# ch4r10t33r/zigz

Measured on AMD Instinct MI355X. Metric: trace steps/sec proved (BabyBear, 2^20 RV64I trace), higher is better.
Workload: dtype u32

## Files before the change

### zigz_amd/csrc/api_commit.cpp

```cpp
#include "api_internal.hpp"

using namespace zk;
using cp::ListCaps;
static_assert(cp::MAX_LEVELS == RUN_MAX_LEVELS && cp::SUMMARY_WORDS == JOB_SUMMARY_WORDS, "commit_plan.hpp restates kernels.hpp");

static void caps_for(zigz_ctx *ctx, size_t npad, unsigned rn, unsigned gn) {
    ListCaps &c = ctx->caps;
    if (c.npad == npad && c.rn == rn && c.gn == gn) return;
    c.npad = npad;
    c.rn = rn;
    c.gn = gn;
    c.g_slabs = false;
    c.g_drops = c.g_skip = c.g_kept = 0;
    memset(c.r_last, 0, sizeof(c.r_last));
    memset(c.g_last, 0, sizeof(c.g_last));
    c.last_dropped = false;
    const LevelLists rw = runs_lists(npad, rn ? rn : 1), gw = cons_lists(npad);
    for (unsigned l = 0; l < RUN_MAX_LEVELS; l++) {
        c.r[l] = l <= rw.top ? (rw.cap[l] / 8 > 256 ? rw.cap[l] / 8 : 256) : 0;
        c.g[l] = l <= gw.top ? 256 : 0;
    }
}

static TreeRef empty_tree_ref(size_t npad) {
// ... 683 lines not shown
    ZIGZ_NOTHROW_BEGIN
    if (job) ZIGZ_ENTER(job->ctx);
    if (!job || !values || !indices || !leaves) return ZIGZ_ERR_INVALID_ARGUMENT;
    zigz_ctx *ctx = job->ctx;
    if (job->state != 1) return ZIGZ_ERR_BAD_STATE;
    const size_t nv = job->nv, ncols = job->ncols;
    if (nv && (!points || !siblings || !dirs)) return ZIGZ_ERR_INVALID_ARGUMENT;
    const size_t sib_b = ncols * nv * 32, leaf_b = ncols * 4, val_b = ncols * 4, dir_b = ncols * nv;
    const size_t out_b = sib_b + leaf_b + val_b + dir_b;
    if (out_b <= PIN_WORDS * 8 / 2 && nv * ncols * 4 + ncols * 8 <= PIN_WORDS * 8 / 2) {
        uint8_t *h = (uint8_t *)ctx->h_pin;
        uint8_t *z_sib = h;
        uint32_t *z_leaf = (uint32_t *)(h + sib_b), *z_val = z_leaf + ncols;
        uint8_t *z_dirs = (uint8_t *)(z_val + ncols);
        uint64_t *h_idx = ctx->h_pin + PIN_WORDS - ncols;
        for (size_t c = 0; c < ncols; c++) {
            h_idx[c] = nv == 0 ? 0 : points[c * nv] % ((uint64_t)1 << nv);
            indices[c] = h_idx[c];
        }
        const bool arena = job->zstride != 0;
        const bool use = job->facts.run_cols && !job->no_eval_skip && (arena || (job->tree.lists && job->col_stride >= job->N));
        EvalSkip skip;
        if (arena) {
            skip.ncols1 = (unsigned)job->ncols1;
            skip.z_in = job->zstride / 4;
            skip.z_changed = job->zstride / 8;
        }
        if (arena || use) memcpy(skip.y_of_col, job->tree.y_of_col, sizeof(skip.y_of_col));
        const unsigned long long *r_ctr = arena ? (const unsigned long long *)((const uint8_t *)ctx->ws[WS_BATCH] + job->off_r_ctr) : ctx->d_run_count;
        if (use) skip.changed = r_ctr + RUN_CHANGED;
        const size_t n_const = use ? job->const_cols : 0;
        if (arena || use) ctx->stats.eval_constant_columns = n_const;
        CHK(timed_begin(ctx, 4));
        if (arena) CHK(dev_eval_radix(ctx, job->d_cols, job->col_stride, ncols, nv, points, z_val, &skip, n_const));
        else CHK(dev_eval_folds(ctx, job->d_cols, job->col_stride, ncols, nv, points, z_val, use ? &skip : nullptr, n_const));
        CHK(timed_end(ctx, 4, &ctx->stats.eval_us));
        const DoneFlag done = done_flag(ctx, 1);
        launch_paths(job->tree, job->tree.npad, (unsigned)nv, job->d_cols, job->col_stride, h_idx, z_sib, z_dirs, z_leaf,
                     job->zstride ? job->ncols1 : ncols, ctx->stream, done);
        HIPCHK(ctx, hipGetLastError());
        if (!(g_sleep_wait.load() && !ctx->timing && sleep_wait(done.flag, done.seq)))
            HIPCHK(ctx, hipStreamSynchronize(ctx->stream));
        if (sib_b) memcpy(siblings, z_sib, sib_b);
        for (size_t c = 0; c < ncols; c++) {
            leaves[c] = z_leaf[c];
            values[c] = z_val[c];
        }
        if (dir_b) memcpy(dirs, z_dirs, dir_b);
        CHK(bind_pool_collect(ctx));
        job->state = 2;
        return ZIGZ_OK;
    }
    if (job->zstride) {
        set_err(ctx, "batched commit job: the openings do not fit the staging buffer");
        return ZIGZ_ERR_INVALID_ARGUMENT;
    }
    void *dv;
    CHK(ws_get(ctx, WS_SCRATCH, ncols * 4 + 64, &dv));
    CHK(timed_begin(ctx, 4));
    CHK(dev_eval_folds(ctx, job->d_cols, job->col_stride, ncols, nv, points, (uint32_t *)dv));
    CHK(timed_end(ctx, 4, &ctx->stats.eval_us));
    std::vector<uint32_t> hv(ncols);
    HIPCHK(ctx, hipMemcpyAsync(hv.data(), dv, ncols * 4, hipMemcpyDeviceToHost, ctx->stream));
    std::vector<uint64_t> idx(ncols);
    for (size_t c = 0; c < ncols; c++) {
        idx[c] = nv == 0 ? 0 : points[c * nv] % ((uint64_t)1 << nv);
        indices[c] = idx[c];
    }
    CHK(open_paths(ctx, job->tree, (unsigned)nv, job->d_cols, job->col_stride, idx.data(), ncols, siblings, dirs, leaves));
    for (size_t c = 0; c < ncols; c++) values[c] = hv[c];
    CHK(bind_pool_collect(ctx));
    job->state = 2;
// ... 90 lines not shown
```

### zigz_amd/csrc/api_internal.hpp

```cpp
#pragma once
#include "zigz_hip.h"

#include <hip/hip_runtime.h>
#include <stdarg.h>
#include <stdio.h>
#include <stdlib.h>
#include <string.h>
#include <time.h>

#include <atomic>
#include <new>
#include <thread>
#include <vector>

#include "commit_plan.hpp"
#include "field.hpp"
#include "kernels.hpp"
#include "sumcheck_host.hpp"

using namespace zk;

enum { WS_IN64 = 0, WS_IN32, WS_OUT32, WS_OUT64, WS_SCRATCH, WS_TREE, WS_FOLD, WS_MISC, WS_COLS, WS_LASSO, WS_DEDUP, WS_WITNESS, WS_RUNS, WS_RUNMETA, WS_CONS, WS_CONSMETA, WS_BATCH, WS_SCBATCH, WS_SCBATCH_IN, WS_VERIFY, WS_OPEN, WS_MLEBATCH, WS_MLEBATCH_PART, WS_MLEBATCH_IN, WS_PRODUCT, WS_PRODUCT_WORK, WS_PRODUCT_IN, WS_EQ, WS_EQ_OUT, WS_SLOTS };

constexpr int KEV_MAX = 72;
// ... 91 lines not shown
            int d_ = -1;                                                             \
            if (hipGetDevice(&d_) != hipSuccess || d_ != (ctx)->device) (void)hipSetDevice((ctx)->device); \
        }                                                                            \
    } while (0)

inline bool is_pow2(size_t n) { return n && !(n & (n - 1)); }
inline size_t ceil_pow2(size_t n) { size_t v = 1; while (v < n) v <<= 1; return v; }
constexpr size_t align256(size_t b) { return (b + 255) & ~(size_t)255; }


#pragma GCC visibility push(hidden)
void set_err(zigz_ctx *ctx, const char *fmt, ...);
zigz_status ws_get(zigz_ctx *ctx, int slot, size_t bytes, void **out);
bool sleep_wait(const unsigned long long *flag, unsigned long long seq);
bool spin_wait(const unsigned long long *flag, unsigned long long seq);
DoneFlag done_flag(zigz_ctx *ctx, int which);
zigz_status wait_published(zigz_ctx *ctx, const DoneFlag &done);
zigz_status pinned(zigz_ctx *ctx, size_t bytes, uint8_t **out);
zigz_status upload_region(zigz_ctx *ctx, size_t bytes, uint8_t **out);
zigz_status log_launch(zigz_ctx *ctx, int cls, uint64_t perms, hipEvent_t start, hipEvent_t stop, hipEvent_t first, double *dur_us);
zigz_status upload_u64(zigz_ctx *ctx, const uint64_t *h_in, size_t n, uint32_t *d_out, bool reduce);
zigz_status download_u64(zigz_ctx *ctx, const uint32_t *d_in, size_t n, uint64_t *h_out);
uint32_t host_to_mont(uint64_t canonical);
zigz_status read_u64(zigz_ctx *ctx, const void *d_src, size_t words, uint64_t *dst);
zigz_status dev_half_sums(zigz_ctx *ctx, const uint32_t *d_in, size_t n, uint64_t out[2]);
zigz_status timed_begin(zigz_ctx *ctx, int ev);
zigz_status timed_end(zigz_ctx *ctx, int ev, double *us_out);
zigz_status bind_launch(zigz_ctx *ctx, const uint32_t *d_in, size_t in_stride, uint32_t *d_out, size_t out_stride,
                               size_t half, size_t ncols, uint32_t r_m, const uint32_t *d_r_m, unsigned long long *d_sums,
                               const SumsLayout *lay = nullptr);
void bind_pool_reset(zigz_ctx *ctx);
zigz_status bind_pool_collect(zigz_ctx *ctx);
zigz_status dev_eval_radix(zigz_ctx *ctx, const uint32_t *d_cols, size_t col_stride, size_t ncols, size_t nv,
                                  const uint64_t *points, uint32_t *d_vals, const EvalSkip *skip = nullptr, size_t n_const = 0);
zigz_status dev_eval_folds(zigz_ctx *ctx, const uint32_t *d_cols, size_t col_stride, size_t ncols, size_t nv,
                                  const uint64_t *points , uint32_t *d_vals, const EvalSkip *skip = nullptr, size_t n_const = 0);
zigz_status sumcheck_core(zigz_ctx *ctx, const uint32_t *d_in, size_t n, uint32_t *d_scratch,
                                 const uint64_t *fixed, uint64_t *rounds, uint64_t *point, uint64_t *final_eval);
zigz_status stage_in(zigz_ctx *ctx, const uint64_t *in, size_t n, uint32_t **d_out);
zigz_status lasso_mapping_check(const uint64_t *table, size_t table_rows, const uint64_t *queries, size_t n_queries, size_t w,
                                const uint64_t *mapping, size_t n_mapping);
struct BuildHints {
    uint64_t small_domain_mask, run_aware_mask, cons_group_mask;
    bool materialize, job;
};
struct BuildResult {
    TreeRef tree;
    uint64_t run_cols, run_dense, sd_cols, cons_hinted, cons_levels_nodes, cons_sd;
};
zigz_status build_trees(zigz_ctx *ctx, const uint32_t *d_vals, size_t val_stride, size_t n_values, size_t npad,
                               uint8_t *d_slab, size_t ncols, bool record, const BuildHints &in, BuildResult *out);
zigz_status keccak_times_collect(zigz_ctx *ctx);
size_t mle_batch_fill(const uint32_t *const *d_tables, const size_t *ns, size_t k, const uint64_t *points, bool reversed,
                      MleBatchTab *tab, uint32_t *f);
zigz_status stage_host_tables(zigz_ctx *ctx, const uint64_t *const *tables, const size_t *ns, size_t count,
                              const std::vector<size_t> &at, uint32_t *h, int slot, const size_t *owner,
                              std::vector<const uint32_t *> &d, size_t *bad_index);
zigz_status mle_eval_pairs_queue(zigz_ctx *ctx, const void *const *tables, bool host_tables, const size_t *ns, size_t m,
                                 const uint64_t *points, bool reversed, const size_t *owner, const uint64_t **results, DoneFlag *done,
                                 size_t *bad_index);
extern std::atomic<int> g_sleep_wait;
#pragma GCC visibility pop

constexpr const char *NOT_CANONICAL_TEXT = "input contains a value >= p (not a canonical BabyBear element)";
template <class Check>
zigz_status host_checks(zigz_ctx *ctx, const uint64_t *const *tables, const size_t *ns, size_t k, size_t *bad_index, Check check) {
    bool value;
    const zigz_status st = checks_in_call_order(tables, ns, k, bad_index, check, &value);
    if (value) set_err(ctx, "%s", NOT_CANONICAL_TEXT);
// ... 20 lines not shown
```

### zigz_amd/csrc/api_mle.cpp

```cpp
#include "api_internal.hpp"

using namespace zk;

zigz_status dev_half_sums(zigz_ctx *ctx, const uint32_t *d_in, size_t n, uint64_t out[2]) {
    const SumsLayout lay = (aligned16(d_in)) ? half_sums_layout(n, 1, 2048) : SumsLayout{2, 1, 0, 1};
    const size_t words = lay.nslots > 1 || lay.col_stride != 2 ? (size_t)lay.nslots * 32 : 2;
    HIPCHK(ctx, hipMemsetAsync(ctx->d_sums, 0, words * 8, ctx->stream));
    launch_half_sums(d_in, n, n, 1, ctx->d_sums, ctx->stream, nullptr, &lay);
    HIPCHK(ctx, hipGetLastError());
    CHK(read_u64(ctx, ctx->d_sums, words, ctx->h_sums));
    out[0] = out[1] = 0;
    for (unsigned k = 0; k < lay.nslots; k++) {
        out[0] += ctx->h_sums[k * lay.slot_stride];
        out[1] += ctx->h_sums[k * lay.slot_stride + lay.bin_stride];
    }
    return ZIGZ_OK;
}

extern "C" zigz_status zigz_dev_mle_half_sums(zigz_ctx *ctx, const uint32_t *d_in, size_t n, uint64_t half_sums[2]) {
    ZIGZ_ENTER(ctx);
    if (!ctx || !d_in || !half_sums) return ZIGZ_ERR_INVALID_ARGUMENT;
    CHK(mle_check(n));
    uint64_t s[2];
    CHK(dev_half_sums(ctx, d_in, n, s));
// ... 80 lines not shown
    CHK(mle_check(n));
    if (n == 1) return ZIGZ_ERR_NO_VARIABLES_TO_FIX;
    if (r >= P) return ZIGZ_ERR_NOT_CANONICAL;
    bind_pool_reset(ctx);
    CHK(timed_begin(ctx, 0));
    CHK(bind_launch(ctx, d_in, n, d_out, n / 2, n / 2, 1, host_to_mont(r), nullptr, nullptr));
    HIPCHK(ctx, hipGetLastError());
    CHK(timed_end(ctx, 0, &ctx->stats.bind_us));
    CHK(bind_pool_collect(ctx));
    ctx->stats.bind_launches = 1;
    return ZIGZ_OK;
}

extern "C" zigz_status zigz_dev_mle_bind_sums(zigz_ctx *ctx, const uint32_t *d_in, size_t n, uint64_t r,
                                              uint32_t *d_out, uint64_t half_sums[2]) {
    ZIGZ_ENTER(ctx);
    if (!ctx || !d_in || !d_out || !half_sums) return ZIGZ_ERR_INVALID_ARGUMENT;
    CHK(mle_check(n));
    if (n == 1) return ZIGZ_ERR_NO_VARIABLES_TO_FIX;
    if (r >= P) return ZIGZ_ERR_NOT_CANONICAL;
    bind_pool_reset(ctx);
    uint64_t s[2];
    CHK(timed_begin(ctx, 0));
    CHK(bind_with_sums(ctx, d_in, n, d_out, host_to_mont(r), s));
    CHK(timed_end(ctx, 0, &ctx->stats.bind_us));
    CHK(bind_pool_collect(ctx));
    ctx->stats.bind_launches = 1;
    half_sums[0] = s[0] % P;
    half_sums[1] = s[1] % P;
    return ZIGZ_OK;
}

zigz_status dev_eval_radix(zigz_ctx *ctx, const uint32_t *d_cols, size_t col_stride, size_t ncols, size_t nv,
                                  const uint64_t *points, uint32_t *d_vals, const EvalSkip *skip, size_t n_const) {
    const size_t N = (size_t)1 << nv;
    const unsigned k2 = 10, k1 = (unsigned)nv - k2;
    const size_t m = (size_t)1 << k2, nb = (size_t)1 << k1;
    const size_t active = skip ? ncols - n_const : ncols;
    const int rloops = active * 2 <= ncols && nb % 16 == 0 ? (active * 4 <= ncols + 3 ? 1 : 2) : 4;
    const size_t groups = radix_fold_groups(nb, rloops);
    if (nv * ncols * 4 > PIN_WORDS * 8 / 2) return ZIGZ_ERR_INVALID_ARGUMENT;
    uint32_t *rt = (uint32_t *)(ctx->h_pin + PIN_WORDS / 2);
    for (size_t c = 0; c < ncols; c++)
        for (size_t j = 0; j < nv; j++) {
            const uint64_t r = points[c * nv + (nv - 1 - j)];
            if (r >= P) return ZIGZ_ERR_NOT_CANONICAL;
            rt[c * nv + j] = host_to_mont(r);
        }
    const uint32_t *d_rt = rt;
    void *ws;
    CHK(ws_get(ctx, WS_FOLD, ncols * (groups * m * 8 + nb * 4 + m * 4 + m * 4) + 256, &ws));
    unsigned long long *d_part = (unsigned long long *)ws;
    uint32_t *d_w1 = (uint32_t *)(d_part + ncols * groups * m), *d_w2 = d_w1 + ncols * nb, *d_t1 = d_w2 + ncols * m;
    launch_eq_weights2(d_rt, nv, k1, d_w1, nb, k2, d_w2, m, ncols, ctx->stream);
    bind_pool_reset(ctx);
    const bool rec = ctx->timing;
    launch_radix_fold(d_cols, col_stride, m, nb, d_w1, nb, d_part, groups * m, ncols, ctx->stream, rec ? ctx->pool[0] : nullptr,
                      rec ? ctx->pool[1] : nullptr, skip, rloops);
    if (rec) {
        ctx->pool_used = 1;
        ctx->pool_is_fold = ctx->active_job != nullptr;
        ctx->pool_bytes = (uint64_t)(ncols - (skip ? n_const : 0)) * (N * 4 + groups * m * 8);
    }
    launch_radix_finalize(d_part, groups * m, groups, d_t1, m, m, 0, nullptr, ncols, ctx->stream, skip);
    launch_weighted_dot(d_t1, m, d_w2, m, m, d_vals, ncols, ctx->stream, skip, d_cols, col_stride);
    HIPCHK(ctx, hipGetLastError());
    return ZIGZ_OK;
}

zigz_status dev_eval_folds(zigz_ctx *ctx, const uint32_t *d_cols, size_t col_stride, size_t ncols, size_t nv,
                                  const uint64_t *points , uint32_t *d_vals, const EvalSkip *skip, size_t n_const) {
    const size_t N = (size_t)1 << nv;
    if (nv == 0) {
        launch_gather_first(d_cols, col_stride, d_vals, ncols, ctx->stream);
        HIPCHK(ctx, hipGetLastError());
        return ZIGZ_OK;
    }
    if (nv >= 14 && nv <= 24 && col_stride % 4 == 0 && aligned16(d_cols) && !ctx->fold_eval)
        return dev_eval_radix(ctx, d_cols, col_stride, ncols, nv, points, d_vals, skip, n_const);
    if (nv * ncols * 4 > PIN_WORDS * 8 / 2) return ZIGZ_ERR_INVALID_ARGUMENT;
    uint32_t *rt = (uint32_t *)(ctx->h_pin + PIN_WORDS / 2);
    for (size_t k = 0; k < nv; k++)
        for (size_t c = 0; c < ncols; c++) {
            uint64_t r = points[c * nv + (nv - 1 - k)];
            if (r >= P) return ZIGZ_ERR_NOT_CANONICAL;
            rt[k * ncols + c] = host_to_mont(r);
        }
    void *d_rt;
    CHK(ws_get(ctx, WS_MISC, nv * ncols * 4 + 64, &d_rt));
    HIPCHK(ctx, hipMemcpyAsync(d_rt, rt, nv * ncols * 4, hipMemcpyHostToDevice, ctx->stream));
    void *fold;
    const size_t a_elems = ncols * (N / 2 < 4 ? 4 : N / 2), b_elems = ncols * (N / 4 < 4 ? 4 : N / 4);
    CHK(ws_get(ctx, WS_FOLD, (a_elems + b_elems) * 4, &fold));
    uint32_t *bufA = (uint32_t *)fold, *bufB = bufA + a_elems;
    bind_pool_reset(ctx);
    const uint32_t *src = d_cols;
    size_t src_stride = col_stride, len = N;
    for (size_t k = 0; k < nv; k++) {
        uint32_t *dst = (k % 2 == 0) ? bufA : bufB;
        size_t half = len / 2;
        size_t dst_stride = half < 4 ? 4 : half;
        CHK(bind_launch(ctx, src, src_stride, dst, dst_stride, half, ncols, 0, (const uint32_t *)d_rt + k * ncols, nullptr));
        src = dst;
        src_stride = dst_stride;
        len = half;
    }
    HIPCHK(ctx, hipGetLastError());
    launch_gather_first(src, src_stride, d_vals, ncols, ctx->stream);
    HIPCHK(ctx, hipGetLastError());
    return ZIGZ_OK;
}

// ... 390 lines not shown
```

### zigz_amd/csrc/kernels.hip

```cpp
#include "kernels.hpp"
#include <hip/hip_ext.h>

#include "field.hpp"
#include "keccak.hpp"
#include "tree_dev.hpp"

namespace zk {

constexpr int UNROLL = 4;
constexpr size_t VEC_MIN_HALF = 4096;


__device__ __forceinline__ void block_add2(unsigned long long s0, unsigned long long s1,
                                           unsigned long long *sums) {
    __shared__ unsigned long long lds[2][TPB / 64];
    s0 = wave_sum(s0);
    s1 = wave_sum(s1);
    int lane = threadIdx.x & 63, wave = threadIdx.x >> 6;
    if (lane == 0) {
        lds[0][wave] = s0;
        lds[1][wave] = s1;
    }
    __syncthreads();
    if (threadIdx.x == 0) {
// ... 227 lines not shown
    const size_t q = (size_t)blockIdx.x * TPB + threadIdx.x;
    if (q * 4 >= m) return;
    const size_t col = blockIdx.z;
    if (eval_skips(skip, col)) return;
    const uint4 *p = reinterpret_cast<const uint4 *>(in + eval_col_off(skip, col, in_stride)) + q;
    const uint32_t *w = w_m + col * w_stride;
    const size_t mq = m / 4;
    unsigned long long lo[4] = {0, 0, 0, 0}, hi[4] = {0, 0, 0, 0};
#pragma unroll 1
    for (int l = 0; l < rloops; l++) {
        const size_t b0 = ((size_t)blockIdx.y * rloops + l) * RB;
        if (!FULL && b0 >= nb) break;
        uint4 v[RB];
#pragma unroll
        for (int j = 0; j < RB; j++) v[j] = ZK_STREAM_LOAD(p + (FULL || b0 + j < nb ? b0 + j : nb - 1) * mq);
#pragma unroll
        for (int j = 0; j < RB; j++) {
            const uint32_t wj = FULL ? w[b0 + j] : (w[b0 + j < nb ? b0 + j : nb - 1] & (b0 + j < nb ? ~0u : 0u));
            const uint32_t e[4] = {v[j].x, v[j].y, v[j].z, v[j].w};
#pragma unroll
            for (int c = 0; c < 4; c++) {
                const unsigned long long pr = (unsigned long long)wj * e[c];
                lo[c] += (uint32_t)pr;
                hi[c] += pr >> 32;
            }
        }
    }
    unsigned long long s[4];
#pragma unroll
    for (int c = 0; c < 4; c++) s[c] = hi[c] + monty_reduce(lo[c]);
    ulonglong2 *o = reinterpret_cast<ulonglong2 *>(part + col * part_col_stride + (size_t)blockIdx.y * m + q * 4);
    o[0] = make_ulonglong2(s[0], s[1]);
    o[1] = make_ulonglong2(s[2], s[3]);
}

size_t radix_fold_groups(size_t nb, int rloops) {
    if (rloops <= 0) rloops = RLOOPS;
    return (nb + (size_t)RB * rloops - 1) / ((size_t)RB * rloops);
}

void launch_radix_fold(const uint32_t *d_in, size_t in_stride, size_t m, size_t nb, const uint32_t *d_w_m,
                       size_t w_stride, unsigned long long *d_part, size_t part_col_stride, size_t ncols, hipStream_t s,
                       hipEvent_t t_start, hipEvent_t t_stop, const EvalSkip *skip, int rloops) {
    if (rloops <= 0) rloops = RLOOPS;
    dim3 grid((unsigned)((m / 4 + TPB - 1) / TPB), (unsigned)radix_fold_groups(nb, rloops), (unsigned)ncols);
    auto kern = nb % ((size_t)RB * rloops) == 0 ? k_radix_fold<true> : k_radix_fold<false>;
    const EvalSkip sk = skip ? *skip : EvalSkip();
    if (t_start && t_stop)
        hipExtLaunchKernelGGL(kern, grid, dim3(TPB), 0, s, t_start, t_stop, 0, d_in, in_stride, m, nb, d_w_m, w_stride,
                              d_part, part_col_stride, sk, rloops);
    else
        hipLaunchKernelGGL(kern, grid, dim3(TPB), 0, s, d_in, in_stride, m, nb, d_w_m, w_stride, d_part, part_col_stride, sk,
                           rloops);
}

__global__ __launch_bounds__(TPB) void k_radix_finalize(const unsigned long long *__restrict__ part, size_t part_col_stride,
                                                        size_t groups, uint32_t *__restrict__ out, size_t out_stride,
                                                        size_t m, unsigned log2_m2, unsigned long long *__restrict__ sums,
                                                        EvalSkip skip, FinalizePublish pub) {
    ZK_PRIO_SMALL();
    __shared__ int s_last;
    const size_t i = (size_t)blockIdx.x * TPB + threadIdx.x;
    const size_t col = blockIdx.z;
    if (eval_skips(skip, col)) return;
    uint32_t v = 0;
    if (i < m) {
// ... 572 lines not shown
    for (unsigned long long w = (unsigned long long)blockIdx.x * (TPB / 64) + (threadIdx.x >> 6); w < count;
         w += (unsigned long long)gridDim.x * (TPB / 64)) {
        const size_t col = cmap.c[todo[2 * w]];
        const size_t i = (size_t)todo[2 * w + 1] * 64 + lane;
        if (i >= npad / 2) continue;
        uint8_t *t = tree + (tmap.n ? (size_t)tmap.c[todo[2 * w]] : col) * tree_stride_nodes * 32;
        const uint32_t *v = vals + col * val_stride;
        const uint64_t v0 = 2 * i < n_values ? v[2 * i] : 0, v1 = 2 * i + 1 < n_values ? v[2 * i + 1] : 0;
        const Digest l0 = sha3_leaf(v0), l1 = sha3_leaf(v1);
        if (write_leaves) {
            store_digest(t, 2 * i, l0);
            store_digest(t, 2 * i + 1, l1);
        }
        store_digest(t, npad + i, sha3_node(l0, l1));
    }
}

void launch_keccak_small_l01(const uint32_t *d_vals, size_t val_stride, size_t n_values, size_t npad, uint8_t *d_tree,
                             size_t tree_stride_nodes, const ColMap &cols, const uint8_t *d_tables,
                             unsigned long long *d_todo_count, uint32_t *d_todo, hipStream_t s, const KTime *kt,
                             bool write_leaves, const unsigned long long *d_only_if, const ColMap *slabs) {
    if (cols.n == 0 || npad < 2) return;
    ColMap tm{};
    if (slabs) tm = *slabs;
    dim3 grid((unsigned)((npad / 2 + TPB - 1) / TPB), (unsigned)cols.n);
    ZK_LAUNCH(kt, k_keccak_small_l01, grid, dim3(TPB), 0, s, d_vals, val_stride, n_values, npad, d_tree, tree_stride_nodes, cols,
              d_tables, d_todo_count, d_todo, write_leaves ? 1 : 0, d_only_if, tm);
    hipLaunchKernelGGL(k_keccak_small_fallback, dim3(512), dim3(TPB), 0, s, d_vals, val_stride, n_values, npad, d_tree,
                       tree_stride_nodes, cols, d_todo_count, d_todo, write_leaves ? 1 : 0, d_only_if, tm);
}

__global__ __launch_bounds__(64) void k_paths(TreeRef t, size_t n_values, unsigned height, const uint32_t *__restrict__ vals,
                                              size_t val_stride, const uint64_t *__restrict__ idx, uint8_t *__restrict__ sib,
                                              uint8_t *__restrict__ dirs, uint32_t *__restrict__ leaf, DoneFlag done) {
    ZK_PRIO_SMALL();
    const size_t col = blockIdx.x;
    const size_t fc = (size_t)blockIdx.z * gridDim.x + col;
    if (t.zstride) vals += (size_t)blockIdx.z * (t.zstride / 4);
    const size_t index = idx[fc];
    const unsigned l = threadIdx.x;
    if (l == 0) leaf[fc] = vals[col * val_stride + index];
    if (l < height) {
        const size_t ci = index >> l;
        const size_t node = ci ^ 1;
        bool virt_leaf = l == 0 && col < 64 && ((t.virtual_leaves >> col) & 1);
        if (l == 0 && col < 64 && ((t.g_sd_mask >> col) & 1) && *t.g_dropped) virt_leaf = true;
        Digest d;
        if (virt_leaf) d = sha3_leaf<false>(node < n_values ? (uint64_t)vals[col * val_stride + node] : 0);
        else d = load_digest_at(node_ptr(t, col, l, node));
        d = canonical_digest(d);
        ulonglong2 *q = reinterpret_cast<ulonglong2 *>(sib + (fc * height + l) * 32);
        q[0] = make_ulonglong2(d.w[0], d.w[1]);
        q[1] = make_ulonglong2(d.w[2], d.w[3]);
        dirs[fc * height + l] = (uint8_t)(ci & 1);
    }
    signal_done(done, gridDim.x * gridDim.z);
}

void launch_paths(const TreeRef &t, size_t n_values, unsigned height, const uint32_t *d_vals, size_t val_stride,
                  const uint64_t *d_idx, uint8_t *d_sib, uint8_t *d_dirs, uint32_t *d_leaf, size_t ncols, hipStream_t s,
                  DoneFlag done) {
    hipLaunchKernelGGL(k_paths, dim3((unsigned)ncols, 1, t.nz ? t.nz : 1), dim3(64), 0, s, t, n_values, height, d_vals, val_stride, d_idx,
                       d_sib, d_dirs, d_leaf, done);
}
__global__ __launch_bounds__(TPB) void k_open_many(TreeRef t, unsigned nv, size_t n_values, const uint32_t *__restrict__ vals,
                                                   size_t val_stride, const mo::Desc *__restrict__ desc, OpenManyZ zf,
                                                   uint8_t *__restrict__ sib, uint8_t *__restrict__ dirs,
                                                   uint64_t *__restrict__ leaf, DoneFlag done) {
    ZK_PRIO_SMALL();
    const unsigned z = blockIdx.z, first = zf.first[z], cnt = zf.first[z + 1] - first;
    if (t.zstride) vals += (size_t)z * (t.zstride / 4);
    const unsigned item = blockIdx.x * TPB + threadIdx.x;
    if (nv == 0) {
        if (item < cnt) {
            const mo::Desc d = desc[first + item];
            leaf[d.off] = vals[(size_t)d.tree * val_stride + d.index];
        }
    } else if (item < cnt * 2 * nv) {
        const unsigned e = item / (2 * nv), r = item - e * 2 * nv, l = r >> 1, half = r & 1;
        const mo::Desc d = desc[first + e];
        const size_t col = d.tree;
        const size_t ci = d.index >> l, node = ci ^ 1;
        bool virt_leaf = l == 0 && col < 64 && ((t.virtual_leaves >> col) & 1);
        if (l == 0 && col < 64 && ((t.g_sd_mask >> col) & 1) && *t.g_dropped) virt_leaf = true;
        uint4 v;
        if (virt_leaf) {
            const Digest g = sha3_leaf<false>(node < n_values ? (uint64_t)vals[col * val_stride + node] : 0);
            const uint64_t a = canonical_word(half ? g.w[2] : g.w[0]), b = canonical_word(half ? g.w[3] : g.w[1]);
            v = make_uint4((uint32_t)a, (uint32_t)(a >> 32), (uint32_t)b, (uint32_t)(b >> 32));
        } else {
            v = canonical_half(node_ptr(t, col, l, node) + half * 16);
        }
        const size_t slot = (size_t)d.off * nv + l;
        *reinterpret_cast<uint4 *>(sib + slot * 32 + half * 16) = v;
        if (!half) {
            dirs[slot] = (uint8_t)(ci & 1);
// ... 215 lines not shown
```

### zigz_amd/csrc/kernels.hpp

```cpp
#pragma once
#include <hip/hip_runtime.h>
#include <stddef.h>
#include <stdint.h>

#include "open_plan.hpp"

namespace zk {

struct KTime {
    hipEvent_t start, stop;
};

inline size_t tree_level_offset(size_t npad, unsigned level) { return 2 * npad - 2 * (npad >> level); }
inline size_t tree_nodes(size_t npad) { return 2 * npad; }

void launch_narrow_u64(const uint64_t *d_in, uint32_t *d_out, size_t n, uint32_t *d_flag, hipStream_t s);
void launch_reduce_u64(const uint64_t *d_in, uint32_t *d_out, size_t n, hipStream_t s);
void launch_witness_rows(const uint64_t *d_rows, size_t num_steps, size_t npad, uint32_t *d_cols, size_t stride,
                         hipStream_t s);
void launch_widen_u32(const uint32_t *d_in, uint64_t *d_out, size_t n, hipStream_t s);
struct TraceStep {
    uint64_t pc, rd_value, mem_addr, mem_value;
    int64_t imm;
    uint8_t opcode, rd, rs1, rs2, funct3, funct7, wr_reg, mem_is_read;
// ... 25 lines not shown
struct Regs32 {
    uint32_t v[32];
};
inline size_t witness_steps_ws_words(size_t npad) {
    const size_t nchunks = (npad + 63) / 64;
    return 65 * nchunks + 64 + 32 * ((nchunks + 255) / 256) + 64;
}
void launch_witness_steps(const TraceStep *d_steps, size_t num_steps, size_t npad, const Regs32 &init, uint32_t *d_ws,
                          uint32_t *d_cols, size_t stride, hipStream_t s, const KTime *kt_expand = nullptr);

struct SumsLayout {
    size_t col_stride, bin_stride, slot_stride;
    unsigned nslots;
};
void launch_bind(const uint32_t *d_in, size_t in_stride, uint32_t *d_out, size_t out_stride, size_t half,
                 size_t ncols, uint32_t r_m, const uint32_t *d_r_m, unsigned long long *d_sums, hipStream_t s,
                 const KTime *kt = nullptr, const SumsLayout *lay = nullptr);
SumsLayout bind_sums_layout(size_t half, size_t ncols, size_t max_words);
bool bind_uses_vec(size_t half, bool with_sums, size_t in_stride, size_t out_stride, const void *in, const void *out);
inline bool aligned16(const void *p) { return ((uintptr_t)p & 15) == 0; }
SumsLayout half_sums_layout(size_t n, size_t ncols, size_t max_words);
void launch_half_sums(const uint32_t *d_in, size_t in_stride, size_t n, size_t ncols,
                      unsigned long long *d_sums, hipStream_t s, const KTime *kt = nullptr, const SumsLayout *lay = nullptr);

void launch_block_sums(const uint32_t *d_in, size_t in_stride, size_t n, unsigned log2_m, size_t ncols,
                       unsigned long long *d_sums, SumsLayout lay, hipStream_t s, const KTime *kt = nullptr);
size_t radix_fold_groups(size_t nb, int rloops = 0);
struct EvalSkip {
    const unsigned long long *changed = nullptr;
    signed char y_of_col[64];
    unsigned ncols1 = 0;
    size_t z_in = 0, z_changed = 0;
};
void launch_radix_fold(const uint32_t *d_in, size_t in_stride, size_t m, size_t nb, const uint32_t *d_w_m,
                       size_t w_stride, unsigned long long *d_part, size_t part_col_stride, size_t ncols, hipStream_t s,
                       hipEvent_t t_start = nullptr, hipEvent_t t_stop = nullptr, const EvalSkip *skip = nullptr, int rloops = 0);
struct DoneFlag;
struct FinalizePublish {
    int kind = 0;
    unsigned n = 0;
    void *h_dst = nullptr;
    unsigned *count = nullptr;
    unsigned long long *flag = nullptr;
    unsigned long long seq = 0;
};
void launch_radix_finalize(const unsigned long long *d_part, size_t part_col_stride, size_t groups, uint32_t *d_out,
                           size_t out_stride, size_t m, unsigned log2_m2, unsigned long long *d_sums, size_t ncols,
                           hipStream_t s, const EvalSkip *skip = nullptr, const FinalizePublish *pub = nullptr);
void launch_eq_weights(const uint32_t *d_r_m, size_t r_stride, unsigned k, uint32_t *d_w_m, size_t w_stride, size_t ncols,
                       hipStream_t s);
void launch_eq_weights2(const uint32_t *d_r_m, size_t r_stride, unsigned kA, uint32_t *d_wA, size_t strideA, unsigned kB,
                        uint32_t *d_wB, size_t strideB, size_t ncols, hipStream_t s);
void launch_weighted_dot(const uint32_t *d_in, size_t in_stride, const uint32_t *d_w_m, size_t w_stride, size_t n,
                         uint32_t *d_out, size_t ncols, hipStream_t s, const EvalSkip *skip = nullptr,
                         const uint32_t *d_cols = nullptr, size_t col_stride = 0);

struct ColMap {
    uint8_t n;
    uint8_t c[64];
};
constexpr unsigned RUN_SEG = 4096;
constexpr unsigned RUN_STAGE_LEVELS = 6;
constexpr unsigned RUN_MAX_LEVELS = 20;
constexpr unsigned RUN_SUBS = 32;
constexpr unsigned RUN_NODE_BITS = 26;
constexpr size_t RUN_MIN_LEAVES = 32768;
// ... 95 lines not shown
    b.vals.zs = b.r_list.zs = b.r_ctr.zs = b.r_stage.zs = b.g_keys.zs = b.g_idx.zs = b.g_rep.zs = b.g_list.zs = b.g_ctr.zs = zs;
}
void launch_runs_structure(const MerkleBuild &b, hipStream_t s, const KTime *kt = nullptr);
void launch_cons_structure(const MerkleBuild &b, hipStream_t s, const KTime *kt = nullptr);
void launch_structure(const MerkleBuild &b, hipStream_t s, bool fused, const KTime *kt = nullptr);
void launch_level_hash(const MerkleBuild &b, unsigned L, hipStream_t s, const KTime *kt = nullptr, size_t expect = 0,
                       bool fused = false);
void launch_fill_virtual(const MerkleBuild &b, hipStream_t s);
void launch_merkle_top(const TreeRef &t, unsigned first_level, unsigned height, size_t ncols, hipStream_t s, const KTime *kt = nullptr);
void launch_keccak_leaves(const uint32_t *d_vals, size_t val_stride, size_t n_values, size_t npad,
                          uint8_t *d_tree, size_t tree_stride_nodes, size_t ncols, hipStream_t s, const KTime *kt = nullptr,
                          const ColMap *cols = nullptr, const ColMap *slabs = nullptr);
void launch_keccak_level(uint8_t *d_tree, size_t tree_stride_nodes, size_t in_off, size_t out_off, size_t n_out,
                         size_t ncols, hipStream_t s, const KTime *kt = nullptr, const ColMap *slabs = nullptr);
constexpr unsigned SD_DOMAIN = 128;
constexpr size_t SD_TABLE_BYTES = (size_t)(SD_DOMAIN + SD_DOMAIN * SD_DOMAIN) * 32;
void launch_sd_tables(uint8_t *d_tables, hipStream_t s);
inline size_t sd_todo_words(size_t npad, size_t ncols) { return 2 * ncols * ((npad / 2 + 63) / 64) + 2; }
void launch_keccak_small_l01(const uint32_t *d_vals, size_t val_stride, size_t n_values, size_t npad, uint8_t *d_tree,
                             size_t tree_stride_nodes, const ColMap &cols, const uint8_t *d_tables,
                             unsigned long long *d_todo_count, uint32_t *d_todo, hipStream_t s, const KTime *kt = nullptr,
                             bool write_leaves = true, const unsigned long long *d_only_if = nullptr,
                             const ColMap *slabs = nullptr);
bool keccak_level_is_wide(size_t n_out, size_t ncols);
struct DoneFlag {
    unsigned *count = nullptr;
    unsigned long long *flag = nullptr;
    unsigned long long seq = 0;
};
void launch_publish_u64(unsigned long long *d_src, size_t n, unsigned long long *h_dst, bool rezero, hipStream_t s, DoneFlag done);
void launch_publish_u32(const uint32_t *d_src, size_t n, uint32_t *h_dst, hipStream_t s, DoneFlag done);
void launch_paths(const TreeRef &t, size_t n_values, unsigned height, const uint32_t *d_vals, size_t val_stride,
                  const uint64_t *d_idx, uint8_t *d_sib, uint8_t *d_dirs, uint32_t *d_leaf, size_t ncols, hipStream_t s,
                  DoneFlag done = DoneFlag());
struct OpenManyZ {
    uint32_t first[33];
};
void launch_open_many(const TreeRef &t, unsigned nv, const uint32_t *d_vals, size_t val_stride, const mo::Desc *d_desc,
                      const OpenManyZ &zf, unsigned nz, uint8_t *d_sib, uint8_t *d_dirs, uint64_t *d_leaf, hipStream_t s,
                      DoneFlag done);
TreeRef slab_tree_ref(uint8_t *d_tree, size_t npad);
void launch_gather_nodes(const uint8_t *d_tree, size_t tree_stride_nodes, size_t node, uint8_t *d_out, size_t ncols,
                         hipStream_t s);
constexpr unsigned JOB_SUMMARY_WORDS = 8 + 2 * RUN_MAX_LEVELS;
void launch_zero_counters(unsigned long long *d_sd_ctr, unsigned long long *d_r_ctr, unsigned long long *d_g_ctr, hipStream_t s,
                          unsigned nz = 0, size_t zstride = 0);
struct ColSrcs {
    const uint32_t *p[32];
};
void launch_gather_cols(const ColSrcs &srcs, unsigned nz, size_t ncols, size_t n, size_t src_stride, uint32_t *d_dst,
                        size_t dst_stride, size_t zstride, hipStream_t s);
void launch_job_summary(const TreeRef &t, unsigned height, uint8_t *d_out, size_t ncols, const unsigned long long *d_r_ctr,
                        const unsigned long long *d_sd_ctr, const unsigned long long *d_g_ctr, hipStream_t s,
                        DoneFlag done = DoneFlag());
void launch_gather_first(const uint32_t *d_in, size_t stride, uint32_t *d_out, size_t ncols, hipStream_t s);
void launch_lasso_fingerprints(const uint32_t *d_rows, size_t rows, size_t width, uint32_t *d_out, hipStream_t s,
                               const KTime *kt = nullptr);
void launch_fill_pattern(uint32_t *d_out, size_t n, uint32_t seed, hipStream_t s);

constexpr unsigned BATCH_WG = 256;
struct BatchTab {
    const uint32_t *in;
    uint32_t *out;
    unsigned long long *part;
    unsigned long long *sums;
    const uint32_t *w;
    uint64_t tail_off;
// ... 178 lines not shown
```

Baseline: 2.286 billion.

## Fuse radix MLE evaluation into one pass and finish it inside the paths kernel

Replaces the multi-launch radix evaluation (eq weights, fold, finalize) with a single kernel. It builds the eq-weight tables in shared memory, streams each column once, and writes one partial sum per block. The final reduction of those partials, plus the copy-through for skipped constant columns, is moved into the existing Merkle-path kernel, so no separate finalize launch is needed. This removes several launches and intermediate buffers per opening. In exchange the weight computation is repeated in every block, and more work is placed inside k_paths.

```diff
diff --git a/zigz_amd/csrc/api_commit.cpp b/zigz_amd/csrc/api_commit.cpp
--- a/zigz_amd/csrc/api_commit.cpp
+++ b/zigz_amd/csrc/api_commit.cpp
@@ -739,12 +739,13 @@
         const size_t n_const = use ? job->const_cols : 0;
         if (arena || use) ctx->stats.eval_constant_columns = n_const;
         CHK(timed_begin(ctx, 4));
-        if (arena) CHK(dev_eval_radix(ctx, job->d_cols, job->col_stride, ncols, nv, points, z_val, &skip, n_const));
-        else CHK(dev_eval_folds(ctx, job->d_cols, job->col_stride, ncols, nv, points, z_val, use ? &skip : nullptr, n_const));
+        EvalFinish fin;
+        if (arena) CHK(dev_eval_radix(ctx, job->d_cols, job->col_stride, ncols, nv, points, z_val, &skip, n_const, &fin));
+        else CHK(dev_eval_folds(ctx, job->d_cols, job->col_stride, ncols, nv, points, z_val, use ? &skip : nullptr, n_const, &fin));
         CHK(timed_end(ctx, 4, &ctx->stats.eval_us));
         const DoneFlag done = done_flag(ctx, 1);
         launch_paths(job->tree, job->tree.npad, (unsigned)nv, job->d_cols, job->col_stride, h_idx, z_sib, z_dirs, z_leaf,
-                     job->zstride ? job->ncols1 : ncols, ctx->stream, done);
+                     job->zstride ? job->ncols1 : ncols, ctx->stream, done, &fin);
         HIPCHK(ctx, hipGetLastError());
         if (!(g_sleep_wait.load() && !ctx->timing && sleep_wait(done.flag, done.seq)))
             HIPCHK(ctx, hipStreamSynchronize(ctx->stream));
diff --git a/zigz_amd/csrc/api_internal.hpp b/zigz_amd/csrc/api_internal.hpp
--- a/zigz_amd/csrc/api_internal.hpp
+++ b/zigz_amd/csrc/api_internal.hpp
@@ -147,9 +147,11 @@
 void bind_pool_reset(zigz_ctx *ctx);
 zigz_status bind_pool_collect(zigz_ctx *ctx);
 zigz_status dev_eval_radix(zigz_ctx *ctx, const uint32_t *d_cols, size_t col_stride, size_t ncols, size_t nv,
-                                  const uint64_t *points, uint32_t *d_vals, const EvalSkip *skip = nullptr, size_t n_const = 0);
+                                  const uint64_t *points, uint32_t *d_vals, const EvalSkip *skip = nullptr, size_t n_const = 0,
+                                  EvalFinish *fin = nullptr);
 zigz_status dev_eval_folds(zigz_ctx *ctx, const uint32_t *d_cols, size_t col_stride, size_t ncols, size_t nv,
-                                  const uint64_t *points , uint32_t *d_vals, const EvalSkip *skip = nullptr, size_t n_const = 0);
+                                  const uint64_t *points , uint32_t *d_vals, const EvalSkip *skip = nullptr, size_t n_const = 0,
+                                  EvalFinish *fin = nullptr);
 zigz_status sumcheck_core(zigz_ctx *ctx, const uint32_t *d_in, size_t n, uint32_t *d_scratch,
                                  const uint64_t *fixed, uint64_t *rounds, uint64_t *point, uint64_t *final_eval);
 zigz_status stage_in(zigz_ctx *ctx, const uint64_t *in, size_t n, uint32_t **d_out);
diff --git a/zigz_amd/csrc/api_mle.cpp b/zigz_amd/csrc/api_mle.cpp
--- a/zigz_amd/csrc/api_mle.cpp
+++ b/zigz_amd/csrc/api_mle.cpp
@@ -136,7 +136,7 @@
 }
 
 zigz_status dev_eval_radix(zigz_ctx *ctx, const uint32_t *d_cols, size_t col_stride, size_t ncols, size_t nv,
-                                  const uint64_t *points, uint32_t *d_vals, const EvalSkip *skip, size_t n_const) {
+                                  const uint64_t *points, uint32_t *d_vals, const EvalSkip *skip, size_t n_const, EvalFinish *fin) {
     const size_t N = (size_t)1 << nv;
     const unsigned k2 = 10, k1 = (unsigned)nv - k2;
     const size_t m = (size_t)1 << k2, nb = (size_t)1 << k1;
@@ -152,6 +152,29 @@
             rt[c * nv + j] = host_to_mont(r);
         }
     const uint32_t *d_rt = rt;
+    const int ro = fin ? eval_onepass_rloops(nb, rloops) : 0;
+    if (ro) {
+        const size_t g1 = nb / ((size_t)16 * ro);
+        void *wp;
+        CHK(ws_get(ctx, WS_FOLD, ncols * g1 * 8 + 256, &wp));
+        bind_pool_reset(ctx);
+        const bool rec1 = ctx->timing;
+        launch_eval_onepass(d_cols, col_stride, (unsigned)nv, d_rt, (unsigned long long *)wp, (unsigned)g1, ncols, ctx->stream,
+                            rec1 ? ctx->pool[0] : nullptr, rec1 ? ctx->pool[1] : nullptr, skip, ro);
+        if (rec1) {
+            ctx->pool_used = 1;
+            ctx->pool_is_fold = ctx->active_job != nullptr;
+            ctx->pool_bytes = (uint64_t)(ncols - (skip ? n_const : 0)) * (N * 4 + g1 * 8);
+        }
+        HIPCHK(ctx, hipGetLastError());
+        fin->part = (const unsigned long long *)wp;
+        fin->groups = (unsigned)g1;
+        fin->skip = skip ? *skip : EvalSkip();
+        fin->out = d_vals;
+        fin->cols = skip ? d_cols : nullptr;
+        fin->col_stride = col_stride;
+        return ZIGZ_OK;
+    }
     void *ws;
     CHK(ws_get(ctx, WS_FOLD, ncols * (groups * m * 8 + nb * 4 + m * 4 + m * 4) + 256, &ws));
     unsigned long long *d_part = (unsigned long long *)ws;
@@ -173,7 +196,8 @@
 }
 
 zigz_status dev_eval_folds(zigz_ctx *ctx, const uint32_t *d_cols, size_t col_stride, size_t ncols, size_t nv,
-                                  const uint64_t *points , uint32_t *d_vals, const EvalSkip *skip, size_t n_const) {
+                                  const uint64_t *points , uint32_t *d_vals, const EvalSkip *skip, size_t n_const,
+                                  EvalFinish *fin) {
     const size_t N = (size_t)1 << nv;
     if (nv == 0) {
         launch_gather_first(d_cols, col_stride, d_vals, ncols, ctx->stream);
@@ -181,7 +205,7 @@
         return ZIGZ_OK;
     }
     if (nv >= 14 && nv <= 24 && col_stride % 4 == 0 && aligned16(d_cols) && !ctx->fold_eval)
-        return dev_eval_radix(ctx, d_cols, col_stride, ncols, nv, points, d_vals, skip, n_const);
+        return dev_eval_radix(ctx, d_cols, col_stride, ncols, nv, points, d_vals, skip, n_const, fin);
     if (nv * ncols * 4 > PIN_WORDS * 8 / 2) return ZIGZ_ERR_INVALID_ARGUMENT;
     uint32_t *rt = (uint32_t *)(ctx->h_pin + PIN_WORDS / 2);
     for (size_t k = 0; k < nv; k++)
diff --git a/zigz_amd/csrc/kernels.hip b/zigz_amd/csrc/kernels.hip
--- a/zigz_amd/csrc/kernels.hip
+++ b/zigz_amd/csrc/kernels.hip
@@ -283,6 +283,92 @@
     ulonglong2 *o = reinterpret_cast<ulonglong2 *>(part + col * part_col_stride + (size_t)blockIdx.y * m + q * 4);
     o[0] = make_ulonglong2(s[0], s[1]);
     o[1] = make_ulonglong2(s[2], s[3]);
+}
+
+__global__ __launch_bounds__(TPB) void k_eval_onepass(const uint32_t *__restrict__ in, size_t in_stride, unsigned nv,
+                                                      const uint32_t *__restrict__ r_m, unsigned long long *__restrict__ part,
+                                                      unsigned groups, EvalSkip skip, int rloops) {
+    ZK_PRIO_SMALL();
+    __shared__ uint32_t s_r[32], s_w1[RB * RLOOPS], s_a[32], s_b[32];
+    __shared__ unsigned long long s_red[TPB / 64];
+    const size_t col = blockIdx.z;
+    if (eval_skips(skip, col)) return;
+    const unsigned t = threadIdx.x, k1 = nv - 10, rows = (unsigned)RB * (unsigned)rloops;
+    const size_t mq = 1024 / 4, row0 = (size_t)blockIdx.y * rows;
+    const uint4 *p = reinterpret_cast<const uint4 *>(in + eval_col_off(skip, col, in_stride)) + t;
+    uint4 v[RB];
+#pragma unroll
+    for (int j = 0; j < RB; j++) v[j] = ZK_STREAM_LOAD(p + (row0 + j) * mq);
+    if (t < nv) s_r[t] = r_m[col * nv + t];
+    __syncthreads();
+    if (t < rows) {
+        const size_t b = row0 + t;
+        uint32_t w = R_MOD_P;
+        for (unsigned j = 0; j < k1; j++) w = mont_mul(w, ((b >> (k1 - 1 - j)) & 1) ? s_r[j] : sub_mod(R_MOD_P, s_r[j]));
+        s_w1[t] = w;
+    } else if (t >= 64 && t < 128) {
+        const unsigned x = t & 31, j0 = k1 + (t >= 96 ? 5 : 0);
+        uint32_t w = R_MOD_P;
+        for (unsigned j = 0; j < 5; j++) w = mont_mul(w, ((x >> (4 - j)) & 1) ? s_r[j0 + j] : sub_mod(R_MOD_P, s_r[j0 + j]));
+        (t >= 96 ? s_b : s_a)[x] = w;
+    }
+    __syncthreads();
+    unsigned long long lo[4] = {0, 0, 0, 0}, hi[4] = {0, 0, 0, 0};
+#pragma unroll 1
+    for (int l = 0; l < rloops; l++) {
+        if (l) {
+#pragma unroll
+            for (int j = 0; j < RB; j++) v[j] = ZK_STREAM_LOAD(p + (row0 + (size_t)l * RB + j) * mq);
+        }
+#pragma unroll
+        for (int j = 0; j < RB; j++) {
+            const uint32_t wj = s_w1[l * RB + j];
+            const uint32_t e[4] = {v[j].x, v[j].y, v[j].z, v[j].w};
+#pragma unroll
+            for (int c = 0; c < 4; c++) {
+                const unsigned long long pr = (unsigned long long)wj * e[c];
+                lo[c] += (uint32_t)pr;
+                hi[c] += pr >> 32;
+            }
+        }
+    }
+    unsigned long long acc = 0;
+#pragma unroll
+    for (int c = 0; c < 4; c++) {
+        const uint32_t sum = (uint32_t)((hi[c] + monty_reduce(lo[c])) % (unsigned long long)P);
+        const unsigned i = 4 * t + c;
+        acc += mont_mul(mont_mul(s_a[i >> 5], s_b[i & 31]), sum);
+    }
+    acc = wave_sum(acc);
+    if ((t & 63) == 0) s_red[t >> 6] = acc;
+    __syncthreads();
+    if (t == 0) {
+        unsigned long long tot = 0;
+        for (int w = 0; w < TPB / 64; w++) tot += s_red[w];
+        part[col * groups + blockIdx.y] = tot;
+    }
+}
+int eval_onepass_rloops(size_t nb, int rloops) {
+#ifdef ZK_EVAL_FOUR_LAUNCHES
+    (void)nb;
+    (void)rloops;
+    return 0;
+#else
+    if (rloops <= 0 || rloops > RLOOPS) rloops = RLOOPS;
+    int r = 1;
+    while (r * 2 <= rloops && nb % ((size_t)RB * r * 2) == 0) r *= 2;
+    return nb % ((size_t)RB * r) == 0 ? r : 0;
+#endif
+}
+void launch_eval_onepass(const uint32_t *d_in, size_t in_stride, unsigned nv, const uint32_t *d_r_m, unsigned long long *d_part,
+                         unsigned groups, size_t ncols, hipStream_t s, hipEvent_t t_start, hipEvent_t t_stop, const EvalSkip *skip,
+                         int rloops) {
+    const dim3 grid(1, groups, (unsigned)ncols);
+    const EvalSkip sk = skip ? *skip : EvalSkip();
+    if (t_start && t_stop)
+        hipExtLaunchKernelGGL(k_eval_onepass, grid, dim3(TPB), 0, s, t_start, t_stop, 0, d_in, in_stride, nv, d_r_m, d_part, groups, sk, rloops);
+    else
+        hipLaunchKernelGGL(k_eval_onepass, grid, dim3(TPB), 0, s, d_in, in_stride, nv, d_r_m, d_part, groups, sk, rloops);
 }
 
 size_t radix_fold_groups(size_t nb, int rloops) {
@@ -921,7 +1007,7 @@
 
 __global__ __launch_bounds__(64) void k_paths(TreeRef t, size_t n_values, unsigned height, const uint32_t *__restrict__ vals,
                                               size_t val_stride, const uint64_t *__restrict__ idx, uint8_t *__restrict__ sib,
-                                              uint8_t *__restrict__ dirs, uint32_t *__restrict__ leaf, DoneFlag done) {
+                                              uint8_t *__restrict__ dirs, uint32_t *__restrict__ leaf, DoneFlag done, EvalFinish fin) {
     ZK_PRIO_SMALL();
     const size_t col = blockIdx.x;
     const size_t fc = (size_t)blockIdx.z * gridDim.x + col;
@@ -943,14 +1029,24 @@
         q[1] = make_ulonglong2(d.w[2], d.w[3]);
         dirs[fc * height + l] = (uint8_t)(ci & 1);
     }
+    if (fin.part) {
+        if (fin.cols && eval_skips(fin.skip, fc)) {
+            if (l == 0) fin.out[fc] = fin.cols[eval_col_off(fin.skip, fc, fin.col_stride)];
+        } else {
+            unsigned long long a = 0;
+            for (unsigned g = l; g < fin.groups; g += 64) a += fin.part[fc * fin.groups + g];
+            a = wave_sum(a);
+            if (l == 0) fin.out[fc] = (uint32_t)(a % (unsigned long long)P);
+        }
+    }
     signal_done(done, gridDim.x * gridDim.z);
 }
 
 void launch_paths(const TreeRef &t, size_t n_values, unsigned height, const uint32_t *d_vals, size_t val_stride,
                   const uint64_t *d_idx, uint8_t *d_sib, uint8_t *d_dirs, uint32_t *d_leaf, size_t ncols, hipStream_t s,
-                  DoneFlag done) {
+                  DoneFlag done, const EvalFinish *fin) {
     hipLaunchKernelGGL(k_paths, dim3((unsigned)ncols, 1, t.nz ? t.nz : 1), dim3(64), 0, s, t, n_values, height, d_vals, val_stride, d_idx,
-                       d_sib, d_dirs, d_leaf, done);
+                       d_sib, d_dirs, d_leaf, done, fin ? *fin : EvalFinish());
 }
 __global__ __launch_bounds__(TPB) void k_open_many(TreeRef t, unsigned nv, size_t n_values, const uint32_t *__restrict__ vals,
                                                    size_t val_stride, const mo::Desc *__restrict__ desc, OpenManyZ zf,
diff --git a/zigz_amd/csrc/kernels.hpp b/zigz_amd/csrc/kernels.hpp
--- a/zigz_amd/csrc/kernels.hpp
+++ b/zigz_amd/csrc/kernels.hpp
@@ -81,6 +81,18 @@
     unsigned ncols1 = 0;
     size_t z_in = 0, z_changed = 0;
 };
+struct EvalFinish {
+    const unsigned long long *part = nullptr;
+    unsigned groups = 0;
+    EvalSkip skip;
+    uint32_t *out = nullptr;
+    const uint32_t *cols = nullptr;
+    size_t col_stride = 0;
+};
+int eval_onepass_rloops(size_t nb, int rloops);
+void launch_eval_onepass(const uint32_t *d_in, size_t in_stride, unsigned nv, const uint32_t *d_r_m, unsigned long long *d_part,
+                         unsigned groups, size_t ncols, hipStream_t s, hipEvent_t t_start, hipEvent_t t_stop, const EvalSkip *skip,
+                         int rloops);
 void launch_radix_fold(const uint32_t *d_in, size_t in_stride, size_t m, size_t nb, const uint32_t *d_w_m,
                        size_t w_stride, unsigned long long *d_part, size_t part_col_stride, size_t ncols, hipStream_t s,
                        hipEvent_t t_start = nullptr, hipEvent_t t_stop = nullptr, const EvalSkip *skip = nullptr, int rloops = 0);
@@ -242,7 +254,7 @@
 void launch_publish_u32(const uint32_t *d_src, size_t n, uint32_t *h_dst, hipStream_t s, DoneFlag done);
 void launch_paths(const TreeRef &t, size_t n_values, unsigned height, const uint32_t *d_vals, size_t val_stride,
                   const uint64_t *d_idx, uint8_t *d_sib, uint8_t *d_dirs, uint32_t *d_leaf, size_t ncols, hipStream_t s,
-                  DoneFlag done = DoneFlag());
+                  DoneFlag done = DoneFlag(), const EvalFinish *fin = nullptr);
 struct OpenManyZ {
     uint32_t first[33];
 };
```

Measured after the change: 2.349 billion, median of 6. 2.7% higher.
